# K1nght/Unified-Unlearning-w-Remain-Geometry

Hardware: AMD Instinct MI355X
Metric: SFR-on unlearning steps/sec, DiT-XL/2 256px bs32/GPU (higher is better)
Workload: dtype bf16

## Files before the change

include/sfron.h:

```cpp
#ifndef SFRON_H
#define SFRON_H
#include <stdint.h>
#ifdef __cplusplus
extern "C" {
#endif

int sfron_abi_version(void);
const char* sfron_build_arch(void);


int sfron_sweep_partials_len(void);

int sfron_sumsq_masked(const float* g, const float* g2, const uint8_t* mask, int64_t n, double* partials, int* nblk_out,
                       void* stream);

int sfron_sumsq_masked_ranges(const float* g, const uint8_t* mask, const int64_t* ranges, int n_ranges, double* partials, void* stream);

int sfron_clip_coef(const double* partials, int nblk, float max_norm, float* stats, void* stream);

int sfron_masked_clip_adam(float* p, const float* g, const float* g2 , float* m, float* v,
                           const uint8_t* mask, const float* stats,
                           int64_t n, double beta1, double beta2, double eps, double step_size, double bc2_sqrt,
                           double decay_mul, uint16_t* w_bf16, float* ema, double ema_decay, int ema_mode, void* stream);

// ... 310 lines not shown

int sfron_reduce_chunks(const float* partials, int groups, int per_group, int D, float* out, int ldout, int accumulate,
                        void* stream);
typedef struct sfron_reduce_item { const float* partials; float* out; int groups, per_group, D, ldout; } sfron_reduce_item;
int sfron_reduce_batch(const sfron_reduce_item* items , int n_items, void* stream);
int sfron_reduce2(const float* p0, const float* p1, int groups, int per_group, int D, float* out0, int ld0, float* out1,
                  int ld1, void* stream);
int sfron_gated_bias_grads(const float* S, const float* gate, int ldg, long gate_stride, long gate_which, int layers, int B,
                           int D, float* out, long out_stride, long out_which0, long out_which1, void* stream);
int sfron_reduce_slots(const float* parts, long slot_stride, int n_slots, int groups, int per_group, int D,
                       float* const* dst_base, const long* dst_layer_stride, const int* dst_ld, void* stream);
int sfron_weighted_reduce(const float* partials, int groups, int per_group, int D, const float* w, int ldw, float* out,
                          void* stream);
int sfron_colsum(const void* X, int is_bf16, int M, int N, int ld, float* partials, int max_partials, float* out,
                 void* stream);

int sfron_timestep_embed(const int64_t* t, int n, int dim, uint16_t* out, int ld, void* stream);
int sfron_silu_fwd(const float* x, int64_t n, uint16_t* y_bf16, void* stream);
int sfron_silu_bwd(const float* dy, const float* x, int64_t n, uint16_t* dx_bf16, float* dx_f32, void* stream);
int sfron_cond_fwd(const float* t_emb, const float* table, const int64_t* y, const uint8_t* drop, int num_classes, int n,
                   int D, float* c, uint16_t* silu_c, void* stream);
int sfron_cond_bwd(const float* d_silu_c, const float* c, const int64_t* y, const uint8_t* drop, int num_classes, int n,
                   int D, float* d_c, float* d_table, void* stream);
int sfron_guard_inputs(const int64_t* y, const int64_t* t, int n, int num_classes, int num_timesteps, int64_t* y_safe, int64_t* t_safe,
                       float* flags, void* stream);
int sfron_guard_finite(const float* a, const float* b, const float* c, const float* d, int n, const float* stats, float* flags, void* stream);
int sfron_latent_sample(const float* moments, const float* eps, int n, int c, int hw, float scale, float* out, void* stream);
int sfron_vae_moments(const float* rows, int ld, int B, int hw, int z2, const float* w, const float* bias, float* moments_f32,
                      uint16_t* moments_f16, const float* eps, float scale, float* latent, void* stream);
int sfron_vae_latent_in(const float* z, int B, int zc, int hw, const float* w, const float* bias, float scale, int c_pad, uint16_t* rows,
                        float* rows_f32, void* stream);
int sfron_patchify(const float* img, int n, int C, int H, int W, int p, int chan_last, uint16_t* rows, int ld, void* stream);
int sfron_unpatchify(const float* rows, int ld, int n, int C, int H, int W, int p, float* img, void* stream);

int sfron_attn_fwd(const uint16_t* qkv, uint16_t* o, float* lse, int B, int T, int H, int hd, void* stream);
int sfron_attn_bwd(const uint16_t* qkv, const uint16_t* o, const uint16_t* d_o, const float* lse, float* delta_scratch,
                   uint16_t* dqkv, int B, int T, int H, int hd, void* stream);
int sfron_attn_bwd_bias_supported(int T);
// ... 97 lines not shown
```

unified-unlearning-w-remain-geometry_amd/_lib.py:

```python
import ctypes
import os
from ctypes import POINTER, c_char_p, c_double, c_float, c_int, c_int64, c_void_p

_HERE = os.path.dirname(os.path.abspath(__file__))
LIB_PATH = os.path.join(_HERE, "libsfron.so")


class SfronError(RuntimeError):
    pass


_lib = None
ABI_VERSION = 16

_P = c_void_p
_S = c_void_p

_PROTOS = {
    "sfron_abi_version": (c_int, []),
    "sfron_build_arch": (c_char_p, []),
    "sfron_sweep_partials_len": (c_int, []),
    "sfron_sumsq_masked": (c_int, [_P, _P, _P, c_int64, _P, POINTER(c_int), _S]),
    "sfron_clip_coef": (c_int, [_P, c_int, c_float, _P, _S]),
    "sfron_masked_clip_adam": (c_int, [_P, _P, _P, _P, _P, _P, _P, c_int64, c_double, c_double, c_double, c_double, c_double,
# ... 56 lines not shown
    "sfron_weighted_reduce": (c_int, [_P, c_int, c_int, c_int, _P, c_int, _P, _S]),
    "sfron_reduce_slots": (c_int, [_P, ctypes.c_long, c_int, c_int, c_int, c_int, POINTER(c_void_p), POINTER(ctypes.c_long),
                                   POINTER(c_int), _S]),
    "sfron_split_finish": (c_int, [_P, c_int64, c_int, c_int, _P, _P, c_int, _S]),
    "sfron_groupnorm_one_launch": (c_int, [c_int, c_int, c_int, c_int]),
    "sfron_groupnorm_fwd_src": (c_int, [_P, _P, _P, _P, c_int, c_int, c_int, c_int, c_float, c_int, _P, c_float, _P, _P, _P, _S]),
    "sfron_groupnorm_bwd_res_src": (c_int, [_P, _P, _P, c_int, _P, _P, _P, _P, c_int, c_int, c_int, c_int, c_int, _P, c_float, _P, c_int, c_int, _P,
                                            c_int, _P, _P, _S]),
    "sfron_groupnorm_bwd_cast_src": (c_int, [_P, _P, _P, c_int, _P, _P, _P, _P, c_int, c_int, c_int, c_int, c_int, _P, c_float, _P, _P, _P, _P, _S]),
    "sfron_reduce_batch": (c_int, [_P, c_int, _S]),
    "sfron_conv_wgrad_scatter_batch": (c_int, [_P, c_int, _S]),
    "sfron_reduce2": (c_int, [_P, _P, c_int, c_int, c_int, _P, c_int, _P, c_int, _S]),
    "sfron_gated_bias_grads": (c_int, [_P, _P, c_int, ctypes.c_long, ctypes.c_long, c_int, c_int, c_int, _P, ctypes.c_long,
                                       ctypes.c_long, ctypes.c_long, _S]),
    "sfron_colsum": (c_int, [_P, c_int, c_int, c_int, c_int, _P, c_int, _P, _S]),
    "sfron_timestep_embed": (c_int, [_P, c_int, c_int, _P, c_int, _S]),
    "sfron_latent_sample": (c_int, [_P, _P, c_int, c_int, c_int, c_float, _P, _S]),
    "sfron_vae_moments": (c_int, [_P, c_int, c_int, c_int, c_int, _P, _P, _P, _P, _P, c_float, _P, _S]),
    "sfron_vae_latent_in": (c_int, [_P, c_int, c_int, c_int, _P, _P, c_float, c_int, _P, _P, _S]),
    "sfron_guard_inputs": (c_int, [_P, _P, c_int, c_int, c_int, _P, _P, _P, _S]),
    "sfron_guard_finite": (c_int, [_P, _P, _P, _P, c_int, _P, _P, _S]),
    "sfron_silu_fwd": (c_int, [_P, c_int64, _P, _S]),
    "sfron_silu_bwd": (c_int, [_P, _P, c_int64, _P, _P, _S]),
    "sfron_cond_fwd": (c_int, [_P, _P, _P, _P, c_int, c_int, c_int, _P, _P, _S]),
    "sfron_cond_bwd": (c_int, [_P, _P, _P, _P, c_int, c_int, c_int, _P, _P, _S]),
    "sfron_patchify": (c_int, [_P, c_int, c_int, c_int, c_int, c_int, c_int, _P, c_int, _S]),
    "sfron_unpatchify": (c_int, [_P, c_int, c_int, c_int, c_int, c_int, c_int, _P, _S]),
    "sfron_attn_fwd": (c_int, [_P, _P, _P, c_int, c_int, c_int, c_int, _S]),
    "sfron_attn_bwd": (c_int, [_P, _P, _P, _P, _P, _P, c_int, c_int, c_int, c_int, _S]),
    "sfron_attn_bwd_form": (c_int, [c_int]),
    "sfron_attn_fwd_form": (c_int, [c_int]),
    "sfron_gemm_loader_waves": (c_int, [c_int]),
    "sfron_attn_bwd_bias_supported": (c_int, [c_int]),
    "sfron_attn_bwd_bias": (c_int, [_P, _P, _P, _P, _P, _P, c_int, c_int, c_int, c_int, _S]),
})


class Fp8GemmDesc(ctypes.Structure):
    _fields_ = [("A", c_void_p), ("B", c_void_p), ("M", c_int), ("N", c_int), ("K", c_int), ("w_scale", c_void_p), ("a_scale", c_float),
                ("epilogue", c_int), ("bias", c_void_p), ("c_bf16", c_void_p), ("ldc_bf16", c_int), ("aux", c_void_p), ("ldaux", c_int),
# ... 233 lines not shown
```

unified-unlearning-w-remain-geometry_amd/csrc/common.h:

```cpp
#pragma once
#include <hip/hip_runtime.h>
#include <stdint.h>

#define SFRON_OK 0
#define SFRON_ERR_ARG 1001
#define SFRON_ERR_UNSUPPORTED 1002

#define SFRON_CHECK_ARG(cond) do { if (!(cond)) return SFRON_ERR_ARG; } while (0)
static inline int64_t sfron_extent(int64_t rows, int64_t ld, int64_t cols, int elem) { return rows > 0 ? ((rows - 1) * ld + cols) * elem : 0; }
static inline bool sfron_fits31(int64_t bytes) { return bytes >= 0 && bytes < (1ll << 31); }

#define SFRON_LAUNCH_STATUS() do { hipError_t e__ = hipGetLastError(); if (e__ != hipSuccess) return (int)e__; } while (0)

typedef __attribute__((ext_vector_type(8))) __bf16 bf16x8;
typedef __attribute__((ext_vector_type(4))) __bf16 bf16x4;
typedef __attribute__((ext_vector_type(2))) __bf16 bf16x2;
typedef __attribute__((ext_vector_type(4))) float f32x4;
typedef __attribute__((ext_vector_type(2))) float f32x2;
typedef unsigned short bf16_raw;

static constexpr int WAVE = 64;

__device__ __forceinline__ float bf2f(__bf16 x) { return (float)x; }
__device__ __forceinline__ __bf16 f2bf(float x) { return (__bf16)x; }
// ... 126 lines not shown

__device__ __forceinline__ uint2 pair_pack8(unsigned a, unsigned b) { permlane16_swap(a, b); return make_uint2(a, b); }
__device__ __forceinline__ void pair_unpack8(uint2 v, unsigned& a, unsigned& b) { a = v.x; b = v.y; permlane16_swap(a, b); }

#include <hip/hip_ext.h>
void sfron_arm_stop_event(hipEvent_t ev);
hipEvent_t sfron_take_stop_event();
#define SFRON_LAUNCH_EV(kernel, grid, block, lds, stream, ...)                                                         \
  do {                                                                                                                 \
    hipEvent_t ev__ = sfron_take_stop_event();                                                                         \
    if (ev__) hipExtLaunchKernelGGL(kernel, grid, block, lds, stream, nullptr, ev__, 0, __VA_ARGS__);                  \
    else hipLaunchKernelGGL(kernel, grid, block, lds, stream, __VA_ARGS__);                                            \
  } while (0)

static inline int cdiv(long a, long b) { return (int)((a + b - 1) / b); }
```

unified-unlearning-w-remain-geometry_amd/csrc/dit_engine.hip:

```cpp
#include <mutex>
#include <vector>
#include "common.h"
#include "../../include/sfron.h"

namespace {

struct Dims {
  int B, C, S, p, D, L, H, hd, F, ncls, fdim, Co;
  int g, T, M, Kp, Po, NM;
};

inline int make_dims(const sfron_dit_cfg* c, Dims& d) {
  if (!c) return SFRON_ERR_ARG;
  d.B = c->batch; d.C = c->in_channels; d.S = c->input_size; d.p = c->patch; d.D = c->hidden; d.L = c->depth;
  d.H = c->heads; d.F = c->mlp_hidden; d.ncls = c->num_classes; d.fdim = c->freq_dim; d.Co = c->out_channels;
  if (d.B <= 0 || d.C <= 0 || d.S <= 0 || d.p <= 0 || d.D <= 0 || d.L <= 0 || d.H <= 0 || d.F <= 0 || d.ncls <= 0) return SFRON_ERR_ARG;
  if (d.S % d.p || d.D % d.H || d.D % 8 || d.F % 8 || d.fdim % 8) return SFRON_ERR_ARG;
  d.hd = d.D / d.H; d.g = d.S / d.p; d.T = d.g * d.g; d.M = d.B * d.T; d.Kp = d.C * d.p * d.p; d.Po = d.p * d.p * d.Co;
  d.NM = (6 * d.L + 2) * d.D;
  if (d.Kp % 8 || d.Po % 8 || (d.T % 64 && d.T > 64) || (d.T & 1)) return SFRON_ERR_UNSUPPORTED;
  if (d.T >= 64 ? (d.hd % 8 || d.hd > 80) : d.hd > 128) return SFRON_ERR_UNSUPPORTED;
  return SFRON_OK;
}

// ... 22 lines not shown
  p.trainable = o;
  p.pos = take((int64_t)d.T * d.D);
  p.total = o;
  return p;
}

struct Workspace {
  __bf16 *patches, *tfreq, *h1s, *sc;
  float *h1, *temb, *c, *mod;
  float* xs;
  __bf16 *xmod1, *qkv, *o, *a1, *xmod2, *hpre, *h, *a2;
  float *mean, *rstd;
  float* lse;
  __bf16* xmodf;
  float* tok;
  float *dx, *dmod, *d_sc, *d_c, *d_h1s, *delta, *part, *csum, *csum2, *slabs, *wslab, *dysum, *bpart, *bpart_qkv;
  float* kslab;
  __bf16 *d_tok, *d_xmod, *d_o, *dmod_bf, *d_c_bf, *d_h1_bf, *dx_bf;
  __bf16 *d_br[2], *d_br2[2], *d_hpre[2], *dqkv[2];
  size_t bytes;
};
constexpr int SPLIT_K_ADA = 256;
constexpr int CSUM_PARTS = 64;

inline int wgrad_splits(int N, int K, int Mred) {
  if (N % 192 || K % 192 || Mred % 64) return 1;
  const int tiles = (N / 192) * (K / 192);
  int s = 224 / tiles;
  if (s > 4) s = 4;
  while (s > 1 && (Mred / 64) % s) --s;
  return s < 1 ? 1 : s;
// ... 35 lines not shown
  w.a2 = (__bf16*)take(L * M * D * 2);
  w.mean = (float*)take((2 * L + 1) * M * 4); w.rstd = (float*)take((2 * L + 1) * M * 4);
  w.lse = (float*)take(L * B * (size_t)d.H * d.T * 4);
  w.xmodf = (__bf16*)take(M * D * 2);
  w.tok = (float*)take(M * (size_t)d.Po * 4);
  w.dx = (float*)take(M * D * 4);
  w.dmod = (float*)take(B * (size_t)d.NM * 4); w.dmod_bf = (__bf16*)take(B * (size_t)d.NM * 2);
  w.d_sc = (float*)take(B * D * 4); w.d_c = (float*)take(B * D * 4); w.d_c_bf = (__bf16*)take(B * D * 2);
  w.d_h1s = (float*)take(B * D * 4); w.d_h1_bf = (__bf16*)take(B * D * 2);
  w.delta = (float*)take(B * (size_t)d.H * d.T * 4);
  w.part = (float*)take((L + 1) * 8 * (size_t)(M / sfron_rows_per_chunk(d.T)) * D * 4);
  const size_t widest = (size_t)(d.F > 3 * d.D ? d.F : 3 * d.D) > (size_t)d.NM ? (size_t)(d.F > 3 * d.D ? d.F : 3 * d.D) : (size_t)d.NM;
  w.csum = (float*)take(CSUM_PARTS * widest * 4);
  w.csum2 = (float*)take(CSUM_PARTS * (size_t)(d.F > 3 * d.D ? d.F : 3 * d.D) * 4);
  w.slabs = (float*)take((size_t)SPLIT_K_ADA * B * D * 4);
  {
    const size_t shapes[4][2] = {{3 * D, D}, {D, D}, {(size_t)d.F, D}, {D, (size_t)d.F}};
    size_t mx = 0;
    for (auto& sh : shapes) { const size_t n = wgrad_splits((int)sh[0], (int)sh[1], (int)M) * sh[0] * sh[1]; mx = n > mx ? n : mx; }
    w.wslab = (float*)take(mx * 4);
  }
  {
    int smax = 1;
    for (const int k : {d.D, d.F, 3 * d.D}) { const int sp = small_m_splits(d.M, d.D, k); smax = sp > smax ? sp : smax; }
    w.kslab = smax > 1 ? (float*)take((size_t)smax * M * D * 4) : nullptr;
  }
  w.dysum = (float*)take((L + 1) * 2 * B * D * 4);
  w.bpart = (float*)take(2 * (size_t)((M + 255) / 256) * (size_t)d.F * 4);
  w.bpart_qkv = (float*)take(2 * B * 3 * D * 4);
  w.d_tok = (__bf16*)take(M * (size_t)d.Po * 2);
// ... 46 lines not shown
  Dims d;
  if (make_dims(cfg, d) != SFRON_OK) return -1;
  return (int64_t)make_ws(d, nullptr).bytes;
}

static int ablate_mask() {
#ifdef SFRON_DEBUG_KNOBS
  static const int m = [] { const char* e = getenv("SFRON_ABLATE"); return e ? atoi(e) : 0; }();
  return m;
#else
  return 0;
#endif
}

struct Probe;
struct Aux { hipStream_t side, side2; hipEvent_t produced[4], consumed[8], done, join2, ada_ready, ada_factors; Probe* probe; const uint8_t* sq_mask; double* sq_partials; int dev;
             const uint8_t* w8t; const float* w8_scales; char* mx_ws;
             char* wg_ws; };

namespace {
struct StreamPair { int dev; hipStream_t a, b; };
std::mutex g_pairs_mu;
std::vector<StreamPair> g_free_pairs;
}

int sfron_aux_create(void** aux) {
  SFRON_CHECK_ARG(aux);
  Aux* a = new Aux{};
  int dev = 0;
  if (hipGetDevice(&dev) != hipSuccess) return (int)hipGetLastError();
  a->dev = dev;
// ... 16 lines not shown
  } else if (hipStreamCreateWithFlags(&a->side, hipStreamNonBlocking) != hipSuccess) return (int)hipGetLastError();
  for (int i = 0; i < 4; ++i)
    if (hipEventCreateWithFlags(&a->produced[i], hipEventDisableTiming) != hipSuccess) return (int)hipGetLastError();
  for (int i = 0; i < 8; ++i)
    if (hipEventCreateWithFlags(&a->consumed[i], hipEventDisableTiming) != hipSuccess) return (int)hipGetLastError();
  if (hipEventCreateWithFlags(&a->done, hipEventDisableTiming) != hipSuccess) return (int)hipGetLastError();
  if (reused) {
  } else if (ablate_mask() & 4) {
    int lo = 0, hi = 0;
    (void)hipDeviceGetStreamPriorityRange(&lo, &hi);
    if (hipStreamCreateWithPriority(&a->side2, hipStreamNonBlocking, lo) != hipSuccess) return (int)hipGetLastError();
  } else if (hipStreamCreateWithFlags(&a->side2, hipStreamNonBlocking) != hipSuccess) return (int)hipGetLastError();
  if (hipEventCreateWithFlags(&a->join2, hipEventDisableTiming) != hipSuccess) return (int)hipGetLastError();
  if (hipEventCreateWithFlags(&a->ada_ready, hipEventDisableTiming) != hipSuccess) return (int)hipGetLastError();
  if (hipEventCreateWithFlags(&a->ada_factors, hipEventDisableTiming) != hipSuccess) return (int)hipGetLastError();
  *aux = a;
  return SFRON_OK;
}
int sfron_aux_set_fp8_dgrad(void* aux, const uint8_t* w8t, const float* w_scales, void* mx_workspace) {
  SFRON_CHECK_ARG(aux && (!w8t || (w_scales && mx_workspace)));
  Aux* a = (Aux*)aux;
  a->w8t = w8t; a->w8_scales = w8t ? w_scales : nullptr; a->mx_ws = w8t ? (char*)mx_workspace : nullptr;
  return SFRON_OK;
}
int sfron_aux_set_fp8_wgrad(void* aux, void* workspace) {
  SFRON_CHECK_ARG(aux && ((uintptr_t)workspace & 15) == 0);
  ((Aux*)aux)->wg_ws = (char*)workspace;
  return SFRON_OK;
}
int sfron_aux_wait_ada(void* aux, void* stream) {
// ... 9 lines not shown
int sfron_aux_wait_ada_factors(void* aux, void* stream) {
  SFRON_CHECK_ARG(aux);
  if (hipStreamWaitEvent((hipStream_t)stream, ((Aux*)aux)->ada_factors, 0) != hipSuccess) return (int)hipGetLastError();
  return SFRON_OK;
}
int sfron_aux_destroy(void* aux) {
  SFRON_CHECK_ARG(aux);
  Aux* a = (Aux*)aux;
  (void)sfron_take_stop_event();
  for (int i = 0; i < 4; ++i) (void)hipEventDestroy(a->produced[i]);
  for (int i = 0; i < 8; ++i) (void)hipEventDestroy(a->consumed[i]);
  (void)hipEventDestroy(a->done);
  (void)hipEventDestroy(a->join2);
  (void)hipEventDestroy(a->ada_ready);
  (void)hipEventDestroy(a->ada_factors);
  if (ablate_mask() & 4) {
    (void)hipStreamDestroy(a->side);
    (void)hipStreamDestroy(a->side2);
  } else {
    (void)hipStreamSynchronize(a->side);
    (void)hipStreamSynchronize(a->side2);
    std::lock_guard<std::mutex> lk(g_pairs_mu);
    g_free_pairs.push_back(StreamPair{a->dev, a->side, a->side2});
  }
  delete a;
  return SFRON_OK;
}

struct Probe { hipEvent_t* ev; int cap, used; };

// ... 425 lines not shown
  const bool f8b = ax && ax->w8t;
  MxWs mx{};
  if (f8b) {
    if (!sfron_fp8_gemm_supported(M, D, 3 * D) || !sfron_fp8_gemm_supported(M, D, D) || !sfron_fp8_gemm_supported(M, d.F, D) ||
        !sfron_fp8_gemm_supported(M, D, d.F) || d.F % 128)
      return SFRON_ERR_UNSUPPORTED;
    (void)mx_ws(d, ax->mx_ws, &mx);
  }
  auto dgrad_fp8 = [&](const uint8_t* a, const uint8_t* a_sc, int64_t w_off, const float* wsc, int N, __bf16* dX) -> int {
    sfron_fp8_dgrad_desc q{};
    q.A = a; q.a_scales = a_sc; q.B = ax->w8t + (w_off - (P.blocks & ~255LL)); q.M = M; q.N = D; q.K = N; q.w_scale = wsc;
    q.epilogue = SFRON_EPI_BF16; q.c_bf16 = (uint16_t*)dX; q.ldc_bf16 = D;
    return sfron_fp8_dgrad(&q, stream);
  };

  RUN(sfron_patchify(d_out, B, d.Co, d.S, d.S, d.p, 1, (uint16_t*)w.d_tok, d.Po, stream));
  RUN(sfron_colsum(w.d_tok, 1, M, d.Po, d.Po, w.csum, CSUM_PARTS, grads + P.fin_b, stream));
  auto small_wgrad = [&](const void* dY, const void* X, int N, int K, float* dW) -> int {
    sfron_gemm_desc q = wgrad_desc(dY, X, M, N, K, dW);
    int sp = M / 256;
    const long cap = (long)SPLIT_K_ADA * B * D / ((long)N * K);
    if (sp > cap) sp = (int)cap;
    if (sp > 64) sp = 64;
    if (sp < 2 || (ablate_mask() & 16)) return sfron_gemm_bf16(&q, stream);
    q.c_f32 = w.slabs; q.split_k = sp; q.split_stride = (long)N * K;
    RUN(sfron_gemm_bf16(&q, stream));
    const int kchunk = cdiv(cdiv(M, sp), 64) * 64;
    return sfron_reduce_chunks(w.slabs, 1, cdiv(M, kchunk), N * K, dW, N * K, 0, stream);
  };
  RUN(small_wgrad(w.d_tok, w.xmodf, d.Po, D, grads + P.fin_w));
  g = dgrad_desc(w.d_tok, wb + P.fin_w, M, d.Po, D);
  g.c_bf16 = (uint16_t*)w.d_xmod; g.ldc_bf16 = D;
  RUN(sfron_gemm_bf16(&g, stream));
  const float* modf = w.mod + (size_t)6 * d.L * D;
  float* dmodf = w.dmod + (size_t)6 * d.L * D;
  {
    const int l = d.L - 1;
    if (fuse) arm(0);
    RUN(ln_gate(w.xs + (size_t)(2 * d.L) * M * D, w.mean + (size_t)(2 * d.L) * M, w.rstd + (size_t)(2 * d.L) * M, modf + D, 0,
                slot(d.L, 3, 0), slot(d.L, 3, 1), w.a2 + (size_t)l * M * D, w.mod + (size_t)l * 6 * D + 5 * D, w.d_br[l & 1],
                slot(l, 0, 0), slot(l, 0, 1)));
  }

  for (int l = d.L - 1; l >= 0; --l) {
// ... 107 lines not shown
    } else {
      RUN(sfron_ln_modulate_bwd((const uint16_t*)w.d_xmod, x0, w.mean, w.rstd, mod + D, NM, T, M, D, w.dx, 1, slot(0, 3, 0),
                                slot(0, 3, 1), stream));
    }
  }
  {
    float* const dst_base[8] = {w.dmod + 5 * D, w.dysum + (size_t)B * D,
                                w.dmod + 3 * D, w.dmod + 4 * D,
                                w.dmod + 2 * D, w.dysum,
                                w.dmod, w.dmod + D};
    const long dst_stride[8] = {6L * D, 2L * B * D, 6L * D, 6L * D, 6L * D, 2L * B * D, 6L * D, 6L * D};
    const int dst_ld[8] = {NM, D, NM, NM, NM, D, NM, NM};
    RUN(sfron_reduce_slots(w.part, slot_stride, d.L * 8, B, per, D, dst_base, dst_stride, dst_ld, stream));
    RUN(sfron_reduce2(slot(d.L, 3, 0), slot(d.L, 3, 1), B, per, D, dmodf, NM, dmodf + D, NM, stream));
  }
  if (ax) { (void)hipEventRecord(ax->done, ax->side); (void)hipStreamWaitEvent(hs, ax->done, 0); }
  if (late_bias) RUN(sfron_gated_bias_grads(w.dysum, w.mod + 2 * D, NM, 6 * D, 3 * D, d.L, B, D, late_bias, 2L * D, 0, D, stream));
  else RUN(sfron_gated_bias_grads(w.dysum, w.mod + 2 * D, NM, 6 * D, 3 * D, d.L, B, D, grads + P.blocks, P.blk_stride, P.o_proj_b,
                                  P.o_fc2_b, stream));
  RUN(sfron_cast_bf16(w.dx, (uint16_t*)w.dx_bf, (int64_t)M * D, stream));
  RUN(sfron_colsum(w.dx, 0, M, D, D, w.csum, CSUM_PARTS, grads + P.pe_b, stream));
  RUN(small_wgrad(w.dx_bf, w.patches, D, d.Kp, grads + P.pe_w));
  RUN(sfron_cast_bf16(w.dmod, (uint16_t*)w.dmod_bf, (int64_t)B * NM, stream));
  RUN(sfron_colsum(w.dmod, 0, B, NM, NM, w.csum, CSUM_PARTS, grads + P.ada_b, stream));
  if (ada_dmod_out && ada_sc_out) {
    if (hipMemcpyAsync(ada_dmod_out, w.dmod_bf, (size_t)B * NM * 2, hipMemcpyDeviceToDevice, hs) != hipSuccess) return (int)hipGetLastError();
    if (hipMemcpyAsync(ada_sc_out, w.sc, (size_t)B * D * 2, hipMemcpyDeviceToDevice, hs) != hipSuccess) return (int)hipGetLastError();
    if (ax) (void)hipEventRecord(ax->ada_factors, hs);
  } else {
    g = wgrad_desc(w.dmod_bf, w.sc, B, NM, D, grads + P.ada_w);
    RUN(sfron_gemm_bf16(&g, stream));
  }
  g = dgrad_desc(w.dmod_bf, wb + P.ada_w, B, NM, D);
  g.epilogue = SFRON_EPI_F32; g.c_f32 = w.slabs; g.ldc_f32 = D; g.split_k = SPLIT_K_ADA; g.split_stride = (long)B * D;
  RUN(sfron_gemm_bf16(&g, stream));
  if (ax) (void)hipEventRecord(ax->ada_ready, hs);
  {
    const int kchunk = cdiv(cdiv(NM, SPLIT_K_ADA), 64) * 64;
    RUN(sfron_reduce_chunks(w.slabs, 1, cdiv(NM, kchunk), B * D, w.d_sc, B * D, 0, stream));
  }
  if (hipMemsetAsync(grads + P.table, 0, (size_t)(d.ncls + 1) * D * sizeof(float), hs) != hipSuccess) return (int)hipGetLastError();
  RUN(sfron_cond_bwd(w.d_sc, w.c, y, drop, d.ncls, B, D, w.d_c, grads + P.table, stream));
  RUN(sfron_cast_bf16(w.d_c, (uint16_t*)w.d_c_bf, (int64_t)B * D, stream));
  RUN(sfron_colsum(w.d_c, 0, B, D, D, w.csum, CSUM_PARTS, grads + P.t2_b, stream));
  g = wgrad_desc(w.d_c_bf, w.h1s, B, D, D, grads + P.t2_w);
  RUN(sfron_gemm_bf16(&g, stream));
  g = dgrad_desc(w.d_c_bf, wb + P.t2_w, B, D, D);
  g.epilogue = SFRON_EPI_F32; g.c_f32 = w.d_h1s; g.ldc_f32 = D;
  RUN(sfron_gemm_bf16(&g, stream));
  RUN(sfron_silu_bwd(w.d_h1s, w.h1, (int64_t)B * D, (uint16_t*)w.d_h1_bf, w.d_sc , stream));
  RUN(sfron_colsum(w.d_sc, 0, B, D, D, w.csum, CSUM_PARTS, grads + P.t0_b, stream));
  g = wgrad_desc(w.d_h1_bf, w.tfreq, B, D, d.fdim, grads + P.t0_w);
  RUN(sfron_gemm_bf16(&g, stream));
  return SFRON_OK;
}
// ... 30 lines not shown
```

unified-unlearning-w-remain-geometry_amd/csrc/embed.hip:

```cpp
#include "common.h"
#include "../../include/sfron.h"

namespace {

constexpr int TPB = 256;

__global__ __launch_bounds__(TPB) void k_timestep_embed(const int64_t* __restrict__ t, int n, int dim, __bf16* __restrict__ out,
                                                        int ld) {
  const int half = dim / 2;
  const int i = blockIdx.x * TPB + threadIdx.x;
  if (i >= n * half) return;
  const int b = i / half, j = i % half;
  const float freq = expf(-9.210340371976184f * (float)j / (float)half);
  const float arg = (float)t[b] * freq;
  out[(size_t)b * ld + j] = f2bf(cosf(arg));
  out[(size_t)b * ld + half + j] = f2bf(sinf(arg));
}

__global__ __launch_bounds__(TPB) void k_silu_fwd(const float* __restrict__ x, int64_t n, __bf16* __restrict__ y) {
  for (int64_t i = (int64_t)blockIdx.x * TPB + threadIdx.x; i < n; i += (int64_t)gridDim.x * TPB) y[i] = f2bf(silu(x[i]));
}
__global__ __launch_bounds__(TPB) void k_silu_bwd(const float* __restrict__ dy, const float* __restrict__ x, int64_t n,
                                                  __bf16* __restrict__ dx_bf16, float* __restrict__ dx_f32) {
  for (int64_t i = (int64_t)blockIdx.x * TPB + threadIdx.x; i < n; i += (int64_t)gridDim.x * TPB) {
    const float g = dy[i] * silu_grad(x[i]);
    if (dx_bf16) dx_bf16[i] = f2bf(g);
    if (dx_f32) dx_f32[i] = g;
  }
}

__global__ __launch_bounds__(TPB) void k_cond_fwd(const float* __restrict__ t_emb, const float* __restrict__ table,
                                                  const int64_t* __restrict__ y, const uint8_t* __restrict__ drop,
                                                  int num_classes, int D, float* __restrict__ c, __bf16* __restrict__ silu_c) {
  const int b = blockIdx.y;
  const int col = blockIdx.x * TPB + threadIdx.x;
  if (col >= D) return;
  const int64_t yb = y[b];
  const int64_t lab = ((drop && drop[b]) || yb < 0 || yb >= num_classes) ? num_classes : yb;
  const float v = t_emb[(size_t)b * D + col] + table[(size_t)lab * D + col];
  c[(size_t)b * D + col] = v;
  silu_c[(size_t)b * D + col] = f2bf(silu(v));
}

constexpr int CB = 32;
__global__ __launch_bounds__(TPB) void k_cond_bwd(const float* __restrict__ d_silu_c, const float* __restrict__ c,
                                                  const int64_t* __restrict__ y, const uint8_t* __restrict__ drop,
                                                  int num_classes, int n, int D, float* __restrict__ d_c,
                                                  float* __restrict__ d_table) {
  __shared__ int s_lab[CB];
  const int col = blockIdx.x * TPB + threadIdx.x;
  for (int b0 = 0; b0 < n; b0 += CB) {
    const int nb = min(CB, n - b0);
    __syncthreads();
    if (threadIdx.x < nb) {
      const int b = b0 + threadIdx.x;
      const int64_t yb = y[b];
      s_lab[threadIdx.x] = ((drop && drop[b]) || yb < 0 || yb >= num_classes) ? num_classes : (int)yb;
    }
    __syncthreads();
    if (col >= D) continue;
    float dv[CB], cv[CB];
#pragma unroll
    for (int i = 0; i < CB; ++i) {
      const int b = b0 + (i < nb ? i : 0);
      dv[i] = d_silu_c[(size_t)b * D + col];
      cv[i] = c[(size_t)b * D + col];
    }
    float g[CB];
#pragma unroll
    for (int i = 0; i < CB; ++i) {
      g[i] = dv[i] * silu_grad(cv[i]);
      if (i < nb) d_c[(size_t)(b0 + i) * D + col] = g[i];
    }
    float tv[CB];
    bool first[CB];
#pragma unroll
    for (int i = 0; i < CB; ++i) {
      const int lab = s_lab[i < nb ? i : 0];
      first[i] = i < nb;
#pragma unroll
      for (int j = 0; j < i; ++j) first[i] = first[i] && s_lab[j] != lab;
      tv[i] = first[i] ? d_table[(size_t)lab * D + col] : 0.f;
    }
#pragma unroll
    for (int i = 0; i < CB; ++i) {
      if (first[i]) {
        const int lab = s_lab[i];
        float v = tv[i];
#pragma unroll
        for (int j = i; j < CB; ++j)
          if (j < nb && s_lab[j] == lab) v += g[j];
        d_table[(size_t)lab * D + col] = v;
      }
    }
  }
}

__global__ __launch_bounds__(TPB) void k_patchify(const float* __restrict__ img, int n, int C, int H, int W, int p,
                                                  int chan_last, __bf16* __restrict__ rows, int ld) {
  const int gw = W / p, gh = H / p, T = gw * gh, K = C * p * p;
  const int64_t total = (int64_t)n * T * K;
  for (int64_t i = (int64_t)blockIdx.x * TPB + threadIdx.x; i < total; i += (int64_t)gridDim.x * TPB) {
    const int k = (int)(i % K);
    const int64_t r = i / K;
    const int tok = (int)(r % T), b = (int)(r / T);
    const int th = tok / gw, tw = tok % gw;
    int c, ph, pw;
    if (chan_last) { c = k % C; const int pq = k / C; ph = pq / p; pw = pq % p; }
    else { c = k / (p * p); const int pq = k % (p * p); ph = pq / p; pw = pq % p; }
// ... 175 lines not shown

int sfron_silu_fwd(const float* x, int64_t n, uint16_t* y_bf16, void* stream) {
  SFRON_CHECK_ARG(x && y_bf16 && n > 0);
  hipLaunchKernelGGL(k_silu_fwd, dim3(grid_for(n)), dim3(TPB), 0, (hipStream_t)stream, x, n, (__bf16*)y_bf16);
  SFRON_LAUNCH_STATUS();
  return SFRON_OK;
}

int sfron_silu_bwd(const float* dy, const float* x, int64_t n, uint16_t* dx_bf16, float* dx_f32, void* stream) {
  SFRON_CHECK_ARG(dy && x && n > 0 && (dx_bf16 || dx_f32));
  hipLaunchKernelGGL(k_silu_bwd, dim3(grid_for(n)), dim3(TPB), 0, (hipStream_t)stream, dy, x, n, (__bf16*)dx_bf16, dx_f32);
  SFRON_LAUNCH_STATUS();
  return SFRON_OK;
}

int sfron_cond_fwd(const float* t_emb, const float* table, const int64_t* y, const uint8_t* drop, int num_classes, int n,
                   int D, float* c, uint16_t* silu_c, void* stream) {
  SFRON_CHECK_ARG(t_emb && table && y && c && silu_c && n > 0 && D > 0 && num_classes > 0);
  hipLaunchKernelGGL(k_cond_fwd, dim3(cdiv(D, TPB), n), dim3(TPB), 0, (hipStream_t)stream, t_emb, table, y, drop, num_classes,
                     D, c, (__bf16*)silu_c);
  SFRON_LAUNCH_STATUS();
  return SFRON_OK;
}

int sfron_cond_bwd(const float* d_silu_c, const float* c, const int64_t* y, const uint8_t* drop, int num_classes, int n,
                   int D, float* d_c, float* d_table, void* stream) {
  SFRON_CHECK_ARG(d_silu_c && c && y && d_c && d_table && n > 0 && D > 0);
  hipLaunchKernelGGL(k_cond_bwd, dim3(cdiv(D, TPB)), dim3(TPB), 0, (hipStream_t)stream, d_silu_c, c, y, drop, num_classes, n,
                     D, d_c, d_table);
  SFRON_LAUNCH_STATUS();
  return SFRON_OK;
}

int sfron_patchify(const float* img, int n, int C, int H, int W, int p, int chan_last, uint16_t* rows, int ld, void* stream) {
  SFRON_CHECK_ARG(img && rows && n > 0 && C > 0 && p > 0 && H % p == 0 && W % p == 0 && ld >= C * p * p);
  hipLaunchKernelGGL(k_patchify, dim3(grid_for((int64_t)n * C * H * W)), dim3(TPB), 0, (hipStream_t)stream, img, n, C, H, W, p,
                     chan_last, (__bf16*)rows, ld);
  SFRON_LAUNCH_STATUS();
  return SFRON_OK;
}

int sfron_unpatchify(const float* rows, int ld, int n, int C, int H, int W, int p, float* img, void* stream) {
  SFRON_CHECK_ARG(img && rows && n > 0 && C > 0 && p > 0 && H % p == 0 && W % p == 0 && ld >= C * p * p);
  hipLaunchKernelGGL(k_unpatchify, dim3(grid_for((int64_t)n * C * H * W)), dim3(TPB), 0, (hipStream_t)stream, rows, ld, n, C, H,
// ... 22 lines not shown
```

unified-unlearning-w-remain-geometry_amd/csrc/norm.hip:

```cpp
#include "common.h"
#include <cstdlib>
#include "../../include/sfron.h"

namespace {

constexpr int TPB = 256;
constexpr int NCH = 5;
constexpr float LN_EPS = 1e-6f;

struct RowRegs { float4 v[NCH]; };

__device__ __forceinline__ void load_row_f32(const float* __restrict__ p, int D4, int lane, RowRegs& r) {
#pragma unroll
  for (int i = 0; i < NCH; ++i) {
    const int c = lane + 64 * i;
    r.v[i] = reinterpret_cast<const float4*>(p)[c < D4 ? c : D4 - 1];
  }
#pragma unroll
  for (int i = 0; i < NCH; ++i)
    if (lane + 64 * i >= D4) r.v[i] = make_float4(0, 0, 0, 0);
}
typedef unsigned int u32x4 __attribute__((ext_vector_type(4)));
typedef unsigned int u32x2 __attribute__((ext_vector_type(2)));
__device__ __forceinline__ __amdgpu_buffer_rsrc_t row_rsrc(const void* p, int bytes) {
// ... 477 lines not shown
  }
  if (wave > 0) {
#pragma unroll
    for (int v = 0; v < VEC; ++v) sh[wave - 1][v][lane] = acc[v];
  }
  __syncthreads();
  if (wave == 0 && col < N) {
#pragma unroll
    for (int v = 0; v < VEC; ++v) {
      acc[v] = ((acc[v] + sh[0][v][lane]) + sh[1][v][lane]) + sh[2][v][lane];
      partials[(size_t)blockIdx.y * N + col + v] = acc[v];
    }
  }
}

struct ChunkPlan { int rpw, combine, rows; };
inline ChunkPlan pick_chunk(int T) {
#ifdef SFRON_DEBUG_KNOBS
  static const int knob = getenv("SFRON_ROW_RPW") ? atoi(getenv("SFRON_ROW_RPW")) : 0;
  if (knob > 0 && T % (4 * knob) == 0) return {knob, 1, 4 * knob};
#endif
  if (T % 32 == 0 && T >= 256) return {8, 1, 32};
  if (T % 16 == 0) return {4, 1, 16};
  if (T % 8 == 0) return {2, 1, 8};
  if (T % 4 == 0) return {1, 1, 4};
  if (T % 2 == 0) return {2, 0, 2};
  return {1, 0, 1};
}

template <bool LN, bool GATE>
// ... 223 lines not shown
}

int sfron_weighted_reduce(const float* partials, int groups, int per_group, int D, const float* w, int ldw, float* out,
                          void* stream) {
  SFRON_CHECK_ARG(partials && out && w && groups > 0 && per_group > 0 && D > 0);
  hipLaunchKernelGGL(k_weighted_reduce, dim3(cdiv(D, TPB)), dim3(TPB), 0, (hipStream_t)stream, partials, groups, per_group,
                     D, w, ldw, out);
  SFRON_LAUNCH_STATUS();
  return SFRON_OK;
}

int sfron_colsum(const void* X, int is_bf16, int M, int N, int ld, float* partials, int max_partials, float* out,
                 void* stream) {
  SFRON_CHECK_ARG(X && partials && out && M > 0 && N > 0 && N % 4 == 0 && ld % 4 == 0 && max_partials > 0);
  SFRON_CHECK_ARG(((uintptr_t)X & 15) == 0);
  int chunks = cdiv(M, 32);
  if (chunks > max_partials) chunks = max_partials;
  const int rpb = cdiv(M, chunks);
  chunks = cdiv(M, rpb);
  hipStream_t hs = (hipStream_t)stream;
  if (is_bf16 && N % 8 == 0 && ld % 8 == 0)
    hipLaunchKernelGGL((k_colsum_partial<__bf16, 8>), dim3(cdiv(N, 512), chunks), dim3(TPB), 0, hs, (const __bf16*)X, M, N, ld, rpb, partials);
  else if (is_bf16)
    hipLaunchKernelGGL((k_colsum_partial<__bf16, 4>), dim3(cdiv(N, 256), chunks), dim3(TPB), 0, hs, (const __bf16*)X, M, N, ld, rpb, partials);
  else
    hipLaunchKernelGGL((k_colsum_partial<float, 4>), dim3(cdiv(N, 256), chunks), dim3(TPB), 0, hs, (const float*)X, M, N, ld, rpb, partials);
  SFRON_LAUNCH_STATUS();
  launch_reduce_chunks(partials, 1, chunks, N, out, N, 0, hs);
  SFRON_LAUNCH_STATUS();
  return SFRON_OK;
}

}
```

Baseline: 16.45.

## Fuse bias colsums into cast/SiLU/cond kernels and offload tail wgrads to side stream

In the backward tail (final layer, patch embed, adaLN, conditioning MLP), bias column sums are fused into the bf16 cast, SiLU-backward and cond-backward kernels, using a ColsumOrder helper that keeps the old chunked summation order. Small wgrad GEMMs, the gated bias grads and several colsums are moved onto the side stream through new events, with a separate split-K slab buffer so they can overlap the main-stream dgrad chain. This is meant to cut the launch count and serialization of many tiny kernels at the end of the step. In exchange it adds extra events, another workspace slab, and kernels that give each column a single thread, which may run with low occupancy.

```diff
diff --git a/include/sfron.h b/include/sfron.h
--- a/include/sfron.h
+++ b/include/sfron.h
@@ -348,14 +348,18 @@
                           void* stream);
 int sfron_colsum(const void* X, int is_bf16, int M, int N, int ld, float* partials, int max_partials, float* out,
                  void* stream);
+int sfron_cast_bf16_colsum(const float* X, int M, int N, uint16_t* dst, float* out, void* stream);
 
 int sfron_timestep_embed(const int64_t* t, int n, int dim, uint16_t* out, int ld, void* stream);
 int sfron_silu_fwd(const float* x, int64_t n, uint16_t* y_bf16, void* stream);
 int sfron_silu_bwd(const float* dy, const float* x, int64_t n, uint16_t* dx_bf16, float* dx_f32, void* stream);
+int sfron_silu_bwd_colsum(const float* dy, const float* x, int n, int D, uint16_t* dx_bf16, float* dx_f32, float* colsum, void* stream);
 int sfron_cond_fwd(const float* t_emb, const float* table, const int64_t* y, const uint8_t* drop, int num_classes, int n,
                    int D, float* c, uint16_t* silu_c, void* stream);
 int sfron_cond_bwd(const float* d_silu_c, const float* c, const int64_t* y, const uint8_t* drop, int num_classes, int n,
                    int D, float* d_c, float* d_table, void* stream);
+int sfron_cond_bwd_fused(const float* d_silu_c, const float* c, const int64_t* y, const uint8_t* drop, int num_classes, int n,
+                         int D, float* d_c, uint16_t* d_c_bf16, float* d_table, float* colsum, void* stream);
 int sfron_guard_inputs(const int64_t* y, const int64_t* t, int n, int num_classes, int num_timesteps, int64_t* y_safe, int64_t* t_safe,
                        float* flags, void* stream);
 int sfron_guard_finite(const float* a, const float* b, const float* c, const float* d, int n, const float* stats, float* flags, void* stream);
diff --git a/unified-unlearning-w-remain-geometry_amd/_lib.py b/unified-unlearning-w-remain-geometry_amd/_lib.py
--- a/unified-unlearning-w-remain-geometry_amd/_lib.py
+++ b/unified-unlearning-w-remain-geometry_amd/_lib.py
@@ -94,6 +94,7 @@
     "sfron_gated_bias_grads": (c_int, [_P, _P, c_int, ctypes.c_long, ctypes.c_long, c_int, c_int, c_int, _P, ctypes.c_long,
                                        ctypes.c_long, ctypes.c_long, _S]),
     "sfron_colsum": (c_int, [_P, c_int, c_int, c_int, c_int, _P, c_int, _P, _S]),
+    "sfron_cast_bf16_colsum": (c_int, [_P, c_int, c_int, _P, _P, _S]),
     "sfron_timestep_embed": (c_int, [_P, c_int, c_int, _P, c_int, _S]),
     "sfron_latent_sample": (c_int, [_P, _P, c_int, c_int, c_int, c_float, _P, _S]),
     "sfron_vae_moments": (c_int, [_P, c_int, c_int, c_int, c_int, _P, _P, _P, _P, _P, c_float, _P, _S]),
@@ -102,8 +103,10 @@
     "sfron_guard_finite": (c_int, [_P, _P, _P, _P, c_int, _P, _P, _S]),
     "sfron_silu_fwd": (c_int, [_P, c_int64, _P, _S]),
     "sfron_silu_bwd": (c_int, [_P, _P, c_int64, _P, _P, _S]),
+    "sfron_silu_bwd_colsum": (c_int, [_P, _P, c_int, c_int, _P, _P, _P, _S]),
     "sfron_cond_fwd": (c_int, [_P, _P, _P, _P, c_int, c_int, c_int, _P, _P, _S]),
     "sfron_cond_bwd": (c_int, [_P, _P, _P, _P, c_int, c_int, c_int, _P, _P, _S]),
+    "sfron_cond_bwd_fused": (c_int, [_P, _P, _P, _P, c_int, c_int, c_int, _P, _P, _P, _P, _S]),
     "sfron_patchify": (c_int, [_P, c_int, c_int, c_int, c_int, c_int, c_int, _P, c_int, _S]),
     "sfron_unpatchify": (c_int, [_P, c_int, c_int, c_int, c_int, c_int, c_int, _P, _S]),
     "sfron_attn_fwd": (c_int, [_P, _P, _P, c_int, c_int, c_int, c_int, _S]),
diff --git a/unified-unlearning-w-remain-geometry_amd/csrc/common.h b/unified-unlearning-w-remain-geometry_amd/csrc/common.h
--- a/unified-unlearning-w-remain-geometry_amd/csrc/common.h
+++ b/unified-unlearning-w-remain-geometry_amd/csrc/common.h
@@ -164,3 +164,23 @@
   } while (0)
 
 static inline int cdiv(long a, long b) { return (int)((a + b - 1) / b); }
+
+constexpr int COLSUM_INLINE_MAX_ROWS = 32 * 63;
+static inline int colsum_chunks(int M, int max_partials) {
+  int chunks = cdiv(M, 32);
+  if (chunks > max_partials) chunks = max_partials;
+  return chunks;
+}
+static inline int colsum_rows_per_chunk(int M, int max_partials) { return cdiv(M, colsum_chunks(M, max_partials)); }
+struct ColsumOrder {
+  float a0, a1, a2, a3, s;
+  int r, rpb;
+  __device__ __forceinline__ explicit ColsumOrder(int rows_per_chunk) : a0(0.f), a1(0.f), a2(0.f), a3(0.f), s(0.f), r(0), rpb(rows_per_chunk) {}
+  __device__ __forceinline__ void close() { s += ((a0 + a1) + a2) + a3; a0 = a1 = a2 = a3 = 0.f; r = 0; }
+  __device__ __forceinline__ void add(float v) {
+    const int w = r & 3;
+    a0 = w == 0 ? a0 + v : a0; a1 = w == 1 ? a1 + v : a1; a2 = w == 2 ? a2 + v : a2; a3 = w == 3 ? a3 + v : a3;
+    if (++r == rpb) close();
+  }
+  __device__ __forceinline__ float total() { if (r) close(); return s; }
+};
diff --git a/unified-unlearning-w-remain-geometry_amd/csrc/dit_engine.hip b/unified-unlearning-w-remain-geometry_amd/csrc/dit_engine.hip
--- a/unified-unlearning-w-remain-geometry_amd/csrc/dit_engine.hip
+++ b/unified-unlearning-w-remain-geometry_amd/csrc/dit_engine.hip
@@ -60,7 +60,7 @@
   float* lse;
   __bf16* xmodf;
   float* tok;
-  float *dx, *dmod, *d_sc, *d_c, *d_h1s, *delta, *part, *csum, *csum2, *slabs, *wslab, *dysum, *bpart, *bpart_qkv;
+  float *dx, *dmod, *d_sc, *d_c, *d_h1s, *delta, *part, *csum, *csum2, *slabs, *slabs2, *wslab, *dysum, *bpart, *bpart_qkv;
   float* kslab;
   __bf16 *d_tok, *d_xmod, *d_o, *dmod_bf, *d_c_bf, *d_h1_bf, *dx_bf;
   __bf16 *d_br[2], *d_br2[2], *d_hpre[2], *dqkv[2];
@@ -126,6 +126,7 @@
   w.csum = (float*)take(CSUM_PARTS * widest * 4);
   w.csum2 = (float*)take(CSUM_PARTS * (size_t)(d.F > 3 * d.D ? d.F : 3 * d.D) * 4);
   w.slabs = (float*)take((size_t)SPLIT_K_ADA * B * D * 4);
+  w.slabs2 = (float*)take((size_t)SPLIT_K_ADA * B * D * 4);
   {
     const size_t shapes[4][2] = {{3 * D, D}, {D, D}, {(size_t)d.F, D}, {D, (size_t)d.F}};
     size_t mx = 0;
@@ -202,7 +203,7 @@
 }
 
 struct Probe;
-struct Aux { hipStream_t side, side2; hipEvent_t produced[4], consumed[8], done, join2, ada_ready, ada_factors; Probe* probe; const uint8_t* sq_mask; double* sq_partials; int dev;
+struct Aux { hipStream_t side, side2; hipEvent_t produced[4], consumed[8], done, join2, ada_ready, ada_factors, ends[3]; Probe* probe; const uint8_t* sq_mask; double* sq_partials; int dev;
              const uint8_t* w8t; const float* w8_scales; char* mx_ws;
              char* wg_ws; };
 
@@ -249,6 +250,8 @@
   if (hipEventCreateWithFlags(&a->join2, hipEventDisableTiming) != hipSuccess) return (int)hipGetLastError();
   if (hipEventCreateWithFlags(&a->ada_ready, hipEventDisableTiming) != hipSuccess) return (int)hipGetLastError();
   if (hipEventCreateWithFlags(&a->ada_factors, hipEventDisableTiming) != hipSuccess) return (int)hipGetLastError();
+  for (int i = 0; i < 3; ++i)
+    if (hipEventCreateWithFlags(&a->ends[i], hipEventDisableTiming) != hipSuccess) return (int)hipGetLastError();
   *aux = a;
   return SFRON_OK;
 }
@@ -288,6 +291,7 @@
   (void)hipEventDestroy(a->join2);
   (void)hipEventDestroy(a->ada_ready);
   (void)hipEventDestroy(a->ada_factors);
+  for (int i = 0; i < 3; ++i) (void)hipEventDestroy(a->ends[i]);
   if (ablate_mask() & 4) {
     (void)hipStreamDestroy(a->side);
     (void)hipStreamDestroy(a->side2);
@@ -743,20 +747,31 @@
     return sfron_fp8_dgrad(&q, stream);
   };
 
+  const bool old_ends = (ablate_mask() & 1024) || B > COLSUM_INLINE_MAX_ROWS;
+  float* const side_csum = ax ? w.csum2 : w.csum;
+  auto hand_to_side = [&](int i) { if (ax) { (void)hipEventRecord(ax->ends[i], hs); (void)hipStreamWaitEvent(ax->side, ax->ends[i], 0); } };
+  if (!old_ends && hipMemsetAsync(grads + P.table, 0, (size_t)(d.ncls + 1) * D * sizeof(float), (hipStream_t)side) != hipSuccess)
+    return (int)hipGetLastError();
   RUN(sfron_patchify(d_out, B, d.Co, d.S, d.S, d.p, 1, (uint16_t*)w.d_tok, d.Po, stream));
-  RUN(sfron_colsum(w.d_tok, 1, M, d.Po, d.Po, w.csum, CSUM_PARTS, grads + P.fin_b, stream));
+  if (old_ends) RUN(sfron_colsum(w.d_tok, 1, M, d.Po, d.Po, w.csum, CSUM_PARTS, grads + P.fin_b, stream));
   auto small_wgrad = [&](const void* dY, const void* X, int N, int K, float* dW) -> int {
+    void* const st = old_ends ? stream : side;
+    float* const slabs = old_ends ? w.slabs : w.slabs2;
     sfron_gemm_desc q = wgrad_desc(dY, X, M, N, K, dW);
     int sp = M / 256;
     const long cap = (long)SPLIT_K_ADA * B * D / ((long)N * K);
     if (sp > cap) sp = (int)cap;
     if (sp > 64) sp = 64;
-    if (sp < 2 || (ablate_mask() & 16)) return sfron_gemm_bf16(&q, stream);
-    q.c_f32 = w.slabs; q.split_k = sp; q.split_stride = (long)N * K;
-    RUN(sfron_gemm_bf16(&q, stream));
+    if (sp < 2 || (ablate_mask() & 16)) return sfron_gemm_bf16(&q, st);
+    q.c_f32 = slabs; q.split_k = sp; q.split_stride = (long)N * K;
+    RUN(sfron_gemm_bf16(&q, st));
     const int kchunk = cdiv(cdiv(M, sp), 64) * 64;
-    return sfron_reduce_chunks(w.slabs, 1, cdiv(M, kchunk), N * K, dW, N * K, 0, stream);
+    return sfron_reduce_chunks(slabs, 1, cdiv(M, kchunk), N * K, dW, N * K, 0, st);
   };
+  if (!old_ends) {
+    hand_to_side(0);
+    RUN(sfron_colsum(w.d_tok, 1, M, d.Po, d.Po, side_csum, CSUM_PARTS, grads + P.fin_b, side));
+  }
   RUN(small_wgrad(w.d_tok, w.xmodf, d.Po, D, grads + P.fin_w));
   g = dgrad_desc(w.d_tok, wb + P.fin_w, M, d.Po, D);
   g.c_bf16 = (uint16_t*)w.d_xmod; g.ldc_bf16 = D;
@@ -894,6 +909,46 @@
     RUN(sfron_reduce_slots(w.part, slot_stride, d.L * 8, B, per, D, dst_base, dst_stride, dst_ld, stream));
     RUN(sfron_reduce2(slot(d.L, 3, 0), slot(d.L, 3, 1), B, per, D, dmodf, NM, dmodf + D, NM, stream));
   }
+  auto ada_dgrad = [&](const void* dmod_bf) -> int {
+    g = dgrad_desc(dmod_bf, wb + P.ada_w, B, NM, D);
+    g.epilogue = SFRON_EPI_F32; g.c_f32 = w.slabs; g.ldc_f32 = D; g.split_k = SPLIT_K_ADA; g.split_stride = (long)B * D;
+    RUN(sfron_gemm_bf16(&g, stream));
+    if (ax) (void)hipEventRecord(ax->ada_ready, hs);
+    const int kchunk = cdiv(cdiv(NM, SPLIT_K_ADA), 64) * 64;
+    return sfron_reduce_chunks(w.slabs, 1, cdiv(NM, kchunk), B * D, w.d_sc, B * D, 0, stream);
+  };
+  if (!old_ends) {
+    hand_to_side(1);
+    if (late_bias) RUN(sfron_gated_bias_grads(w.dysum, w.mod + 2 * D, NM, 6 * D, 3 * D, d.L, B, D, late_bias, 2L * D, 0, D, side));
+    else RUN(sfron_gated_bias_grads(w.dysum, w.mod + 2 * D, NM, 6 * D, 3 * D, d.L, B, D, grads + P.blocks, P.blk_stride, P.o_proj_b,
+                                    P.o_fc2_b, side));
+    RUN(sfron_cast_bf16(w.dx, (uint16_t*)w.dx_bf, (int64_t)M * D, side));
+    RUN(sfron_colsum(w.dx, 0, M, D, D, side_csum, CSUM_PARTS, grads + P.pe_b, side));
+    RUN(small_wgrad(w.dx_bf, w.patches, D, d.Kp, grads + P.pe_w));
+    const bool factors = ada_dmod_out && ada_sc_out;
+    uint16_t* const dmod_bf = factors ? ada_dmod_out : (uint16_t*)w.dmod_bf;
+    RUN(sfron_cast_bf16_colsum(w.dmod, B, NM, dmod_bf, grads + P.ada_b, stream));
+    if (factors) {
+      if (hipMemcpyAsync(ada_sc_out, w.sc, (size_t)B * D * 2, hipMemcpyDeviceToDevice, hs) != hipSuccess) return (int)hipGetLastError();
+      if (ax) (void)hipEventRecord(ax->ada_factors, hs);
+    } else {
+      g = wgrad_desc(dmod_bf, w.sc, B, NM, D, grads + P.ada_w);
+      RUN(sfron_gemm_bf16(&g, stream));
+    }
+    RUN(ada_dgrad(dmod_bf));
+    RUN(sfron_cond_bwd_fused(w.d_sc, w.c, y, drop, d.ncls, B, D, w.d_c, (uint16_t*)w.d_c_bf, grads + P.table, grads + P.t2_b, stream));
+    hand_to_side(2);
+    g = wgrad_desc(w.d_c_bf, w.h1s, B, D, D, grads + P.t2_w);
+    RUN(sfron_gemm_bf16(&g, side));
+    g = dgrad_desc(w.d_c_bf, wb + P.t2_w, B, D, D);
+    g.epilogue = SFRON_EPI_F32; g.c_f32 = w.d_h1s; g.ldc_f32 = D;
+    RUN(sfron_gemm_bf16(&g, stream));
+    RUN(sfron_silu_bwd_colsum(w.d_h1s, w.h1, B, D, (uint16_t*)w.d_h1_bf, nullptr, grads + P.t0_b, stream));
+    g = wgrad_desc(w.d_h1_bf, w.tfreq, B, D, d.fdim, grads + P.t0_w);
+    RUN(sfron_gemm_bf16(&g, stream));
+    if (ax) { (void)hipEventRecord(ax->done, ax->side); (void)hipStreamWaitEvent(hs, ax->done, 0); }
+    return SFRON_OK;
+  }
   if (ax) { (void)hipEventRecord(ax->done, ax->side); (void)hipStreamWaitEvent(hs, ax->done, 0); }
   if (late_bias) RUN(sfron_gated_bias_grads(w.dysum, w.mod + 2 * D, NM, 6 * D, 3 * D, d.L, B, D, late_bias, 2L * D, 0, D, stream));
   else RUN(sfron_gated_bias_grads(w.dysum, w.mod + 2 * D, NM, 6 * D, 3 * D, d.L, B, D, grads + P.blocks, P.blk_stride, P.o_proj_b,
@@ -911,14 +966,7 @@
     g = wgrad_desc(w.dmod_bf, w.sc, B, NM, D, grads + P.ada_w);
     RUN(sfron_gemm_bf16(&g, stream));
   }
-  g = dgrad_desc(w.dmod_bf, wb + P.ada_w, B, NM, D);
-  g.epilogue = SFRON_EPI_F32; g.c_f32 = w.slabs; g.ldc_f32 = D; g.split_k = SPLIT_K_ADA; g.split_stride = (long)B * D;
-  RUN(sfron_gemm_bf16(&g, stream));
-  if (ax) (void)hipEventRecord(ax->ada_ready, hs);
-  {
-    const int kchunk = cdiv(cdiv(NM, SPLIT_K_ADA), 64) * 64;
-    RUN(sfron_reduce_chunks(w.slabs, 1, cdiv(NM, kchunk), B * D, w.d_sc, B * D, 0, stream));
-  }
+  RUN(ada_dgrad(w.dmod_bf));
   if (hipMemsetAsync(grads + P.table, 0, (size_t)(d.ncls + 1) * D * sizeof(float), hs) != hipSuccess) return (int)hipGetLastError();
   RUN(sfron_cond_bwd(w.d_sc, w.c, y, drop, d.ncls, B, D, w.d_c, grads + P.table, stream));
   RUN(sfron_cast_bf16(w.d_c, (uint16_t*)w.d_c_bf, (int64_t)B * D, stream));
diff --git a/unified-unlearning-w-remain-geometry_amd/csrc/embed.hip b/unified-unlearning-w-remain-geometry_amd/csrc/embed.hip
--- a/unified-unlearning-w-remain-geometry_amd/csrc/embed.hip
+++ b/unified-unlearning-w-remain-geometry_amd/csrc/embed.hip
@@ -27,6 +27,33 @@
     if (dx_bf16) dx_bf16[i] = f2bf(g);
     if (dx_f32) dx_f32[i] = g;
   }
+}
+
+__global__ __launch_bounds__(64) void k_silu_bwd_colsum(const float* __restrict__ dy, const float* __restrict__ x, int n, int D,
+                                                        int rows_per_chunk, __bf16* __restrict__ dx_bf16, float* __restrict__ dx_f32,
+                                                        float* __restrict__ colsum) {
+  const int col = blockIdx.x * 64 + threadIdx.x;
+  if (col >= D) return;
+  ColsumOrder sum(rows_per_chunk);
+  constexpr int U = 32;
+  for (int b0 = 0; b0 < n; b0 += U) {
+    float dv[U], xv[U];
+#pragma unroll
+    for (int i = 0; i < U; ++i) {
+      const int b = b0 + i < n ? b0 + i : n - 1;
+      dv[i] = dy[(size_t)b * D + col];
+      xv[i] = x[(size_t)b * D + col];
+    }
+#pragma unroll
+    for (int i = 0; i < U; ++i) {
+      if (b0 + i >= n) break;
+      const float g = dv[i] * silu_grad(xv[i]);
+      if (dx_bf16) dx_bf16[(size_t)(b0 + i) * D + col] = f2bf(g);
+      if (dx_f32) dx_f32[(size_t)(b0 + i) * D + col] = g;
+      sum.add(g);
+    }
+  }
+  colsum[col] = sum.total();
 }
 
 __global__ __launch_bounds__(TPB) void k_cond_fwd(const float* __restrict__ t_emb, const float* __restrict__ table,
@@ -43,12 +70,16 @@
 }
 
 constexpr int CB = 32;
-__global__ __launch_bounds__(TPB) void k_cond_bwd(const float* __restrict__ d_silu_c, const float* __restrict__ c,
-                                                  const int64_t* __restrict__ y, const uint8_t* __restrict__ drop,
-                                                  int num_classes, int n, int D, float* __restrict__ d_c,
-                                                  float* __restrict__ d_table) {
+template <int NT, bool FUSED>
+__global__ __launch_bounds__(NT) void k_cond_bwd(const float* __restrict__ d_silu_c, const float* __restrict__ c,
+                                                 const int64_t* __restrict__ y, const uint8_t* __restrict__ drop,
+                                                 int num_classes, int n, int D, float* __restrict__ d_c,
+                                                 float* __restrict__ d_table, __bf16* __restrict__ d_c_bf16,
+                                                 float* __restrict__ colsum, int rows_per_chunk) {
+  static_assert(NT >= CB, "the first CB threads stage the labels");
   __shared__ int s_lab[CB];
-  const int col = blockIdx.x * TPB + threadIdx.x;
+  const int col = blockIdx.x * NT + threadIdx.x;
+  ColsumOrder sum(rows_per_chunk);
   for (int b0 = 0; b0 < n; b0 += CB) {
     const int nb = min(CB, n - b0);
     __syncthreads();
@@ -71,6 +102,9 @@
     for (int i = 0; i < CB; ++i) {
       g[i] = dv[i] * silu_grad(cv[i]);
       if (i < nb) d_c[(size_t)(b0 + i) * D + col] = g[i];
+      if constexpr (FUSED) {
+        if (i < nb) { d_c_bf16[(size_t)(b0 + i) * D + col] = f2bf(g[i]); sum.add(g[i]); }
+      }
     }
     float tv[CB];
     bool first[CB];
@@ -93,6 +127,9 @@
         d_table[(size_t)lab * D + col] = v;
       }
     }
+  }
+  if constexpr (FUSED) {
+    if (col < D) colsum[col] = sum.total();
   }
 }
 
@@ -298,6 +335,15 @@
   return SFRON_OK;
 }
 
+int sfron_silu_bwd_colsum(const float* dy, const float* x, int n, int D, uint16_t* dx_bf16, float* dx_f32, float* colsum, void* stream) {
+  SFRON_CHECK_ARG(dy && x && colsum && n > 0 && D > 0);
+  if (n > COLSUM_INLINE_MAX_ROWS) return SFRON_ERR_UNSUPPORTED;
+  hipLaunchKernelGGL(k_silu_bwd_colsum, dim3(cdiv(D, 64)), dim3(64), 0, (hipStream_t)stream, dy, x, n, D, colsum_rows_per_chunk(n, 64),
+                     (__bf16*)dx_bf16, dx_f32, colsum);
+  SFRON_LAUNCH_STATUS();
+  return SFRON_OK;
+}
+
 int sfron_cond_fwd(const float* t_emb, const float* table, const int64_t* y, const uint8_t* drop, int num_classes, int n,
                    int D, float* c, uint16_t* silu_c, void* stream) {
   SFRON_CHECK_ARG(t_emb && table && y && c && silu_c && n > 0 && D > 0 && num_classes > 0);
@@ -310,8 +356,18 @@
 int sfron_cond_bwd(const float* d_silu_c, const float* c, const int64_t* y, const uint8_t* drop, int num_classes, int n,
                    int D, float* d_c, float* d_table, void* stream) {
   SFRON_CHECK_ARG(d_silu_c && c && y && d_c && d_table && n > 0 && D > 0);
-  hipLaunchKernelGGL(k_cond_bwd, dim3(cdiv(D, TPB)), dim3(TPB), 0, (hipStream_t)stream, d_silu_c, c, y, drop, num_classes, n,
-                     D, d_c, d_table);
+  hipLaunchKernelGGL((k_cond_bwd<TPB, false>), dim3(cdiv(D, TPB)), dim3(TPB), 0, (hipStream_t)stream, d_silu_c, c, y, drop, num_classes, n,
+                     D, d_c, d_table, (__bf16*)nullptr, (float*)nullptr, 1);
+  SFRON_LAUNCH_STATUS();
+  return SFRON_OK;
+}
+
+int sfron_cond_bwd_fused(const float* d_silu_c, const float* c, const int64_t* y, const uint8_t* drop, int num_classes, int n,
+                         int D, float* d_c, uint16_t* d_c_bf16, float* d_table, float* colsum, void* stream) {
+  SFRON_CHECK_ARG(d_silu_c && c && y && d_c && d_c_bf16 && d_table && colsum && n > 0 && D > 0);
+  if (n > COLSUM_INLINE_MAX_ROWS) return SFRON_ERR_UNSUPPORTED;
+  hipLaunchKernelGGL((k_cond_bwd<64, true>), dim3(cdiv(D, 64)), dim3(64), 0, (hipStream_t)stream, d_silu_c, c, y, drop, num_classes, n,
+                     D, d_c, d_table, (__bf16*)d_c_bf16, colsum, colsum_rows_per_chunk(n, 64));
   SFRON_LAUNCH_STATUS();
   return SFRON_OK;
 }
diff --git a/unified-unlearning-w-remain-geometry_amd/csrc/norm.hip b/unified-unlearning-w-remain-geometry_amd/csrc/norm.hip
--- a/unified-unlearning-w-remain-geometry_amd/csrc/norm.hip
+++ b/unified-unlearning-w-remain-geometry_amd/csrc/norm.hip
@@ -515,6 +515,51 @@
   }
 }
 
+__global__ __launch_bounds__(TPB) void k_cast_colsum(const float* __restrict__ X, int M, int N, int rows_per_chunk,
+                                                     __bf16* __restrict__ dst, float* __restrict__ out) {
+  __shared__ float sh[3][4][64];
+  const int lane = threadIdx.x & 63, wave = threadIdx.x >> 6;
+  const int col = (blockIdx.x * 64 + lane) * 4;
+  float tot[4] = {0.f, 0.f, 0.f, 0.f};
+  for (int r0 = 0; r0 < M; r0 += rows_per_chunk) {
+    const int r1 = min(M, r0 + rows_per_chunk);
+    float acc[4] = {0.f, 0.f, 0.f, 0.f};
+    if (col < N) {
+      const float* p = X + col;
+      int r = r0 + wave;
+      for (; r + 12 < r1; r += 16) {
+        float4 q[4];
+#pragma unroll
+        for (int u = 0; u < 4; ++u) q[u] = *reinterpret_cast<const float4*>(p + (size_t)(r + 4 * u) * N);
+#pragma unroll
+        for (int u = 0; u < 4; ++u) {
+          acc[0] += q[u].x; acc[1] += q[u].y; acc[2] += q[u].z; acc[3] += q[u].w;
+          *reinterpret_cast<bf16x4*>(dst + (size_t)(r + 4 * u) * N + col) = bf16x4{f2bf(q[u].x), f2bf(q[u].y), f2bf(q[u].z), f2bf(q[u].w)};
+        }
+      }
+      for (; r < r1; r += 4) {
+        const float4 q = *reinterpret_cast<const float4*>(p + (size_t)r * N);
+        acc[0] += q.x; acc[1] += q.y; acc[2] += q.z; acc[3] += q.w;
+        *reinterpret_cast<bf16x4*>(dst + (size_t)r * N + col) = bf16x4{f2bf(q.x), f2bf(q.y), f2bf(q.z), f2bf(q.w)};
+      }
+    }
+    __syncthreads();
+    if (wave > 0) {
+#pragma unroll
+      for (int v = 0; v < 4; ++v) sh[wave - 1][v][lane] = acc[v];
+    }
+    __syncthreads();
+    if (wave == 0) {
+#pragma unroll
+      for (int v = 0; v < 4; ++v) tot[v] += ((acc[v] + sh[0][v][lane]) + sh[1][v][lane]) + sh[2][v][lane];
+    }
+  }
+  if (wave == 0 && col < N) {
+#pragma unroll
+    for (int v = 0; v < 4; ++v) out[col + v] = tot[v];
+  }
+}
+
 struct ChunkPlan { int rpw, combine, rows; };
 inline ChunkPlan pick_chunk(int T) {
 #ifdef SFRON_DEBUG_KNOBS
@@ -768,10 +813,8 @@
                  void* stream) {
   SFRON_CHECK_ARG(X && partials && out && M > 0 && N > 0 && N % 4 == 0 && ld % 4 == 0 && max_partials > 0);
   SFRON_CHECK_ARG(((uintptr_t)X & 15) == 0);
-  int chunks = cdiv(M, 32);
-  if (chunks > max_partials) chunks = max_partials;
-  const int rpb = cdiv(M, chunks);
-  chunks = cdiv(M, rpb);
+  const int rpb = colsum_rows_per_chunk(M, max_partials);
+  const int chunks = cdiv(M, rpb);
   hipStream_t hs = (hipStream_t)stream;
   if (is_bf16 && N % 8 == 0 && ld % 8 == 0)
     hipLaunchKernelGGL((k_colsum_partial<__bf16, 8>), dim3(cdiv(N, 512), chunks), dim3(TPB), 0, hs, (const __bf16*)X, M, N, ld, rpb, partials);
@@ -785,4 +828,14 @@
   return SFRON_OK;
 }
 
-}
+int sfron_cast_bf16_colsum(const float* X, int M, int N, uint16_t* dst, float* out, void* stream) {
+  SFRON_CHECK_ARG(X && dst && out && M > 0 && N > 0 && N % 4 == 0);
+  SFRON_CHECK_ARG(((uintptr_t)X & 15) == 0 && ((uintptr_t)dst & 7) == 0);
+  if (M > COLSUM_INLINE_MAX_ROWS) return SFRON_ERR_UNSUPPORTED;
+  hipLaunchKernelGGL(k_cast_colsum, dim3(cdiv(N, 256)), dim3(TPB), 0, (hipStream_t)stream, X, M, N, colsum_rows_per_chunk(M, 64),
+                     (__bf16*)dst, out);
+  SFRON_LAUNCH_STATUS();
+  return SFRON_OK;
+}
+
+}
```

Result: no change. 16.40 (-0.3%).
